# renly/Actor-Critic-Algs-on-Tensorflow

Hardware: AMD Instinct MI355X
Metric: env-steps/sec (whole node) A2C Atari-CNN 32 vec-envs/GPU at 1/2/4/8 MI355X (higher is better)
Workload: dtype bf16; 1 GPU; model=Nature-CNN actor-critic (3 conv + fc512, 1.69M params), global_batch=160, seq_len=5, envs_per_gpu=32, algo=A2C (RMSprop 7e-4, n-step returns, grad-norm 0.5), parallelism=dp1, engine=native, hipgraph=True, dp_schedule=single, grad_bucket_dtype=fp32, dp_world1=False

## Files before the change

### csrc/kernels/cnn_fused.hip

```cpp
#include <cstdlib>

#include "common.h"
#include "cnn_head.h"
#include "launch_api.h"
#include "pong_env.h"

namespace aca {

constexpr int T_THREADS = 256;
constexpr int OBS_BYTES = 4 * 84 * 84;
constexpr int W1_LD = 256 + 8;
constexpr int Y1_ROWS = 400, Y1_C = 32;
constexpr int Y2_ROWS = 81, Y2_C = 64;
constexpr int Y1_LD = 40, Y2_LD = 80;
constexpr int Y3_ROWS = 49, Y3_C = 64;

typedef short short8v __attribute__((ext_vector_type(8)));

__device__ __forceinline__ uint2 u8x4_to_bf16(uint32_t w) {
  uint2 r;
  r.x = (__float_as_uint((float)(w & 0xFF)) >> 16) | (__float_as_uint((float)((w >> 8) & 0xFF)) & 0xFFFF0000u);
  r.y = (__float_as_uint((float)((w >> 16) & 0xFF)) >> 16) | (__float_as_uint((float)(w >> 24)) & 0xFFFF0000u);
  return r;
}
// ... 99 lines not shown
  static constexpr int oia = PART == 1 ? 40 : 0, oib = PART == 0 ? 40 : 84;
  static constexpr int P1 = (c1b - c1a) * 20, T1 = (P1 + 15) / 16;
  static constexpr int P2 = (c2b - c2a) * 9, T2 = (P2 + 15) / 16;
  static constexpr int P3 = (c3b - c3a) * 7, T3 = (P3 + 15) / 16;
  static_assert(c1b <= 20 && ib <= 84 && oia * 84 % 16 == 0, "row ranges");
};
static_assert(EnvRows<-1>::P1 == 400 && EnvRows<-1>::P2 == 81 && EnvRows<-1>::P3 == 49, "whole env");
static_assert(EnvRows<0>::T1 == 15 && EnvRows<1>::T1 == 18 && EnvRows<0>::ib == 52 && EnvRows<1>::ia == 24 &&
              EnvRows<0>::c1b >= EnvRows<0>::o1b && EnvRows<1>::c1a <= EnvRows<1>::o1a &&
              EnvRows<0>::c2b >= EnvRows<0>::o2b && EnvRows<1>::c2a <= EnvRows<1>::o2a &&
              EnvRows<0>::ib >= EnvRows<0>::oib && EnvRows<1>::ia <= EnvRows<1>::oia, "halves own what they compute");
constexpr int E1P_ELEMS = 14 * E1_W * Y1_LD;

template <int PART, bool FRAG = false>
__device__ __forceinline__ void trunk_env_convs(const uint8_t* __restrict__ s_obs8, u16* __restrict__ s_y1,
                                                u16* __restrict__ s_y2, int e, const bf16x8 (&bw)[2][8],
                                                const bf16x8 (&bw2)[16], const u16* __restrict__ W3, float bias0,
                                                float bias1, float bias2, float bias3, u16* __restrict__ y1g,
                                                u16* __restrict__ y2g, u16* __restrict__ y3g, float scale,
                                                uint64_t* __restrict__ stamps = nullptr) {
  using R = EnvRows<PART>;
  constexpr int NW = 4;
  const int tid = threadIdx.x, lane = tid & 63, wid = tid >> 6;
  const int l16 = lane & 15, lg = lane >> 4;
  const int n2 = wid * 16 + l16;
  for (int mt = wid; mt < R::T1; mt += NW) {
    floatx4 acc0 = {0.f, 0.f, 0.f, 0.f}, acc1 = {0.f, 0.f, 0.f, 0.f};
    const int m = min(mt * 16 + l16, R::P1 - 1);
    const int oh = R::c1a + m / 20, ow = m % 20;
#pragma unroll
    for (int ks = 0; ks < 8; ++ks) {
      const int k = ks * 32 + lg * 8;
      const int c = k >> 6, i = (k >> 3) & 7;
      const uint8_t* p = s_obs8 + (c * 84 + oh * 4 + i) * 84 + ow * 4;
      const uint2 lo = u8x4_to_bf16(*reinterpret_cast<const uint32_t*>(p));
      const uint2 hi = u8x4_to_bf16(*reinterpret_cast<const uint32_t*>(p + 4));
      const bf16x8 a = __builtin_bit_cast(bf16x8, make_uint4(lo.x, lo.y, hi.x, hi.y));
      acc0 = __builtin_amdgcn_mfma_f32_16x16x32_bf16(a, bw[0][ks], acc0, 0, 0, 0);
      acc1 = __builtin_amdgcn_mfma_f32_16x16x32_bf16(a, bw[1][ks], acc1, 0, 0, 0);
    }
#pragma unroll
    for (int r = 0; r < 4; ++r) {
      const int row = mt * 16 + lg * 4 + r;
      if (R::P1 % 16 == 0 || row < R::P1) {
        const u16 v0 = f2bf(fmaxf(acc0[r] * scale + bias0, 0.f));
        const u16 v1 = f2bf(fmaxf(acc1[r] * scale + bias1, 0.f));
        const int lr = row / 20, col = row % 20;
        const int px1 = lr * E1_W + col;
        s_y1[px1 * Y1_LD + l16] = v0;
        s_y1[px1 * Y1_LD + 16 + l16] = v1;
        if (PART < 0 || (R::c1a + lr >= R::o1a && R::c1a + lr < R::o1b)) {
          const size_t g = (size_t)e * Y1_ROWS + R::c1a * 20 + row;
          y1g[g * Y1_C + l16] = v0;
          y1g[g * Y1_C + 16 + l16] = v1;
        }
      }
    }
  }
  bf16x8 bw3[18];
  load_w3<FRAG>(W3, bw3);
  __syncthreads();
  stamp(stamps, 5);
  {
    floatx4 acc[R::T2];
#pragma unroll
    for (int mt = 0; mt < R::T2; ++mt) acc[mt] = floatx4{0.f, 0.f, 0.f, 0.f};
#pragma unroll
    for (int ks = 0; ks < 16; ++ks) {
      const int k = ks * 32 + lg * 8;
      const int i = k >> 7, j = (k >> 5) & 3, c0 = k & 31;
#pragma unroll
      for (int mt = 0; mt < R::T2; ++mt) {
        const int m = min(mt * 16 + l16, R::P2 - 1);
        const int oh = m / 9, ow = m - oh * 9;
        const bf16x8 a = *reinterpret_cast<const bf16x8*>(s_y1 + ((oh * 2 + i) * E1_W + ow * 2 + j) * Y1_LD + c0);
        acc[mt] = __builtin_amdgcn_mfma_f32_16x16x32_bf16(a, bw2[ks], acc[mt], 0, 0, 0);
      }
    }
#pragma unroll
    for (int mt = 0; mt < R::T2; ++mt) {
#pragma unroll
      for (int r = 0; r < 4; ++r) {
        const int row = mt * 16 + lg * 4 + r;
        if (row < R::P2) {
          const u16 v = f2bf(fmaxf(acc[mt][r] + bias2, 0.f));
          const int lr = row / 9;
          s_y2[(lr * E2_W + row % 9) * Y2_LD + n2] = v;
          if (PART < 0 || (R::c2a + lr >= R::o2a && R::c2a + lr < R::o2b))
            y2g[((size_t)e * Y2_ROWS + R::c2a * 9 + row) * Y2_C + n2] = v;
        }
      }
    }
  }
  __syncthreads();
  stamp(stamps, 6);
  {
    floatx4 acc[R::T3];
#pragma unroll
    for (int mt = 0; mt < R::T3; ++mt) acc[mt] = floatx4{0.f, 0.f, 0.f, 0.f};
#pragma unroll
    for (int ks = 0; ks < 18; ++ks) {
      const int k = ks * 32 + lg * 8;
      const int i = k / 192, j = (k >> 6) % 3, c0 = k & 63;
#pragma unroll
      for (int mt = 0; mt < R::T3; ++mt) {
        const int m = min(mt * 16 + l16, R::P3 - 1);
        const int oh = m / 7, ow = m - oh * 7;
        const bf16x8 a = *reinterpret_cast<const bf16x8*>(s_y2 + ((oh + i) * E2_W + ow + j) * Y2_LD + c0);
        acc[mt] = __builtin_amdgcn_mfma_f32_16x16x32_bf16(a, bw3[ks], acc[mt], 0, 0, 0);
      }
    }
#pragma unroll
    for (int mt = 0; mt < R::T3; ++mt) {
#pragma unroll
      for (int r = 0; r < 4; ++r) {
        const int row = mt * 16 + lg * 4 + r;
        if (row < R::P3)
          y3g[((size_t)e * Y3_ROWS + R::c3a * 7 + row) * Y3_C + n2] = f2bf(fmaxf(acc[mt][r] + bias3, 0.f));
      }
    }
  }
  stamp(stamps, 7);
}

__device__ __forceinline__ void w1_lds_dma(const u16* __restrict__ W1, u16* dst_lds) {
  const int lane = threadIdx.x & 63, wid = threadIdx.x >> 6, nw = blockDim.x >> 6;
  for (int blk = wid; blk < 16; blk += nw) {
    const int q = blk * 64 + lane, row = q >> 5, lc = (q & 31) ^ (row & 15);
    __builtin_amdgcn_global_load_lds(reinterpret_cast<const uint4*>(W1) + row * 32 + lc,
                                     (__attribute__((address_space(3))) void*)(dst_lds + blk * 512), 16, 0, 0);
  }
}
__device__ __forceinline__ void w1_frags_from_lds(const u16* __restrict__ s_w, bf16x8 (&bw)[2][8]) {
  const int lane = threadIdx.x & 63, l16 = lane & 15, lg = lane >> 4;
#pragma unroll
  for (int nt = 0; nt < 2; ++nt)
#pragma unroll
    for (int ks = 0; ks < 8; ++ks) {
      const int row = nt * 16 + l16, pc = (ks * 4 + lg) ^ (row & 15);
      bw[nt][ks] = *reinterpret_cast<const bf16x8*>(s_w + row * 256 + pc * 8);
    }
}

constexpr int E1T_ELEMS = 20 * 20 * Y1_C;
__device__ __forceinline__ int e1t_addr(int h, int w, int ch) {
  return (h * 20 + (w & 1) * 10 + (w >> 1)) * Y1_C + (((ch >> 3) ^ (((h >> 1) & 1) << 1)) << 3) + (ch & 7);
}
constexpr int OB16_ELEMS = 4 * 84 * 84;
static_assert(E1T_ELEMS + E2_ELEMS <= OB16_ELEMS && Y3_ROWS * Y3_C <= E1T_ELEMS, "y1 + y2 (+ y3) reuse the image");

template <bool FRAG>
__global__ void __launch_bounds__(256) cnn_trunk_fwd_s16_kernel(
    const uint8_t* __restrict__ obs, const u16* __restrict__ W1, const float* __restrict__ b1,
    const u16* __restrict__ W2, const float* __restrict__ b2, const u16* __restrict__ W3,
    const float* __restrict__ b3, u16* __restrict__ y1g, u16* __restrict__ y2g, u16* __restrict__ y3g,
    float scale, uint8_t* __restrict__ shift_out, const int64_t* __restrict__ obs_idx) {
  __shared__ __attribute__((aligned(16))) u16 s_img[OB16_ELEMS];
  u16* const s_y1 = s_img;
  u16* const s_y2 = s_img + E1T_ELEMS;
  u16* const s_y3 = s_img;
  const int e = blockIdx.x;
  const int tid = threadIdx.x, lane = tid & 63, wid = tid >> 6;
  const int l16 = lane & 15, lg = lane >> 4;
  const int n2 = wid * 16 + l16;
  constexpr int NCH = OBS_BYTES / 16, PER = (NCH + 255) / 256;
  const uint4* src = reinterpret_cast<const uint4*>(obs + (size_t)(obs_idx ? obs_idx[e] : e) * OBS_BYTES);
  uint4 v[PER];
#pragma unroll
  for (int u = 0; u < PER; ++u) v[u] = src[min(tid + u * 256, NCH - 1)];
  bf16x8 bw[2][8];
  if constexpr (FRAG) frag_w1(W1, bw);
  else trunk_env_w1(W1, bw);
  const float bias0 = b1[l16], bias1 = b1[16 + l16], bias2 = b2[n2], bias3 = b3[n2];
#pragma unroll
  for (int u = 0; u < PER; ++u) {
    const int i = tid + u * 256;
    if (i < NCH) {
      const uint2 a = u8x4_to_bf16(v[u].x), b = u8x4_to_bf16(v[u].y);
      const uint2 c = u8x4_to_bf16(v[u].z), d = u8x4_to_bf16(v[u].w);
      uint4* dst = reinterpret_cast<uint4*>(s_img) + 2 * i;
      dst[0] = make_uint4(a.x, a.y, b.x, b.y);
      dst[1] = make_uint4(c.x, c.y, d.x, d.y);
      if (shift_out && i >= NCH / 4)
        reinterpret_cast<uint4*>(shift_out + (size_t)e * OBS_BYTES)[i - NCH / 4] = v[u];
    }
  }
  __syncthreads();
  constexpr int MT1 = 7;
  uint32_t yr[MT1][4];
#pragma unroll
  for (int q = 0; q < MT1; ++q) {
    const int mt = wid + 4 * q;
    if (mt < 25) {
      floatx4 acc0 = {0.f, 0.f, 0.f, 0.f}, acc1 = {0.f, 0.f, 0.f, 0.f};
      const int m = mt * 16 + l16;
      const int oh = m / 20, ow = m - oh * 20;
#pragma unroll
      for (int ks = 0; ks < 8; ++ks) {
        const int k = ks * 32 + lg * 8;
        const int c = k >> 6, i = (k >> 3) & 7;
        const u16* p = s_img + (c * 84 + oh * 4 + i) * 84 + ow * 4;
        const uint2 lo = *reinterpret_cast<const uint2*>(p), hi = *reinterpret_cast<const uint2*>(p + 4);
        const bf16x8 a = __builtin_bit_cast(bf16x8, make_uint4(lo.x, lo.y, hi.x, hi.y));
        acc0 = __builtin_amdgcn_mfma_f32_16x16x32_bf16(a, bw[0][ks], acc0, 0, 0, 0);
        acc1 = __builtin_amdgcn_mfma_f32_16x16x32_bf16(a, bw[1][ks], acc1, 0, 0, 0);
      }
#pragma unroll
      for (int r = 0; r < 4; ++r)
        yr[q][r] = (uint32_t)f2bf(fmaxf(acc0[r] * scale + bias0, 0.f)) |
                   ((uint32_t)f2bf(fmaxf(acc1[r] * scale + bias1, 0.f)) << 16);
    }
  }
  bf16x8 bw2[16];
  load_w2<FRAG>(W2, bw2);
  __syncthreads();
#pragma unroll
  for (int q = 0; q < MT1; ++q) {
    const int mt = wid + 4 * q;
    if (mt < 25)
#pragma unroll
      for (int r = 0; r < 4; ++r) {
        const int row = mt * 16 + lg * 4 + r, h = row / 20, w = row - h * 20;
        s_y1[e1t_addr(h, w, l16)] = (u16)(yr[q][r] & 0xFFFFu);
        s_y1[e1t_addr(h, w, 16 + l16)] = (u16)(yr[q][r] >> 16);
      }
  }
  __syncthreads();
  for (int i = tid; i < Y1_ROWS * 4; i += 256) {
    const int p = i >> 2, cq = i & 3, h = p / 20, w = p - h * 20;
    *reinterpret_cast<uint4*>(y1g + ((size_t)e * Y1_ROWS + p) * Y1_C + cq * 8) =
        *reinterpret_cast<const uint4*>(s_y1 + e1t_addr(h, w, cq * 8));
  }
  {
    floatx4 acc[6];
#pragma unroll
    for (int mt = 0; mt < 6; ++mt) acc[mt] = floatx4{0.f, 0.f, 0.f, 0.f};
#pragma unroll
    for (int ks = 0; ks < 16; ++ks) {
      const int k = ks * 32 + lg * 8;
      const int i = k >> 7, j = (k >> 5) & 3, c0 = k & 31;
#pragma unroll
      for (int mt = 0; mt < 6; ++mt) {
        const int m = min(mt * 16 + l16, Y2_ROWS - 1);
        const int oh = m / 9, ow = m - oh * 9;
        const bf16x8 a = *reinterpret_cast<const bf16x8*>(s_y1 + e1t_addr(oh * 2 + i, ow * 2 + j, c0));
        acc[mt] = __builtin_amdgcn_mfma_f32_16x16x32_bf16(a, bw2[ks], acc[mt], 0, 0, 0);
      }
    }
#pragma unroll
    for (int mt = 0; mt < 6; ++mt)
#pragma unroll
      for (int r = 0; r < 4; ++r) {
        const int row = mt * 16 + lg * 4 + r;
        if (row < Y2_ROWS)
          s_y2[((row / 9) * E2_W + row % 9) * Y2_LD + n2] = f2bf(fmaxf(acc[mt][r] + bias2, 0.f));
      }
  }
  bf16x8 bw3[18];
  load_w3<FRAG>(W3, bw3);
  __syncthreads();
  for (int i = tid; i < Y2_ROWS * 8; i += 256) {
    const int p = i >> 3, cq = i & 7;
    *reinterpret_cast<uint4*>(y2g + ((size_t)e * Y2_ROWS + p) * Y2_C + cq * 8) =
        *reinterpret_cast<const uint4*>(s_y2 + ((p / 9) * E2_W + p % 9) * Y2_LD + cq * 8);
  }
  {
    floatx4 acc[4];
#pragma unroll
    for (int mt = 0; mt < 4; ++mt) acc[mt] = floatx4{0.f, 0.f, 0.f, 0.f};
#pragma unroll
    for (int ks = 0; ks < 18; ++ks) {
      const int k = ks * 32 + lg * 8;
      const int i = k / 192, j = (k >> 6) % 3, c0 = k & 63;
#pragma unroll
      for (int mt = 0; mt < 4; ++mt) {
        const int m = min(mt * 16 + l16, Y3_ROWS - 1);
        const int oh = m / 7, ow = m - oh * 7;
        const bf16x8 a = *reinterpret_cast<const bf16x8*>(s_y2 + ((oh + i) * E2_W + ow + j) * Y2_LD + c0);
        acc[mt] = __builtin_amdgcn_mfma_f32_16x16x32_bf16(a, bw3[ks], acc[mt], 0, 0, 0);
      }
    }
#pragma unroll
    for (int mt = 0; mt < 4; ++mt)
#pragma unroll
      for (int r = 0; r < 4; ++r) {
        const int row = mt * 16 + lg * 4 + r;
        if (row < Y3_ROWS) s_y3[row * Y3_C + n2] = f2bf(fmaxf(acc[mt][r] + bias3, 0.f));
      }
  }
  __syncthreads();
  for (int i = tid; i < Y3_ROWS * 8; i += 256)
    reinterpret_cast<uint4*>(y3g + (size_t)e * Y3_ROWS * Y3_C)[i] = reinterpret_cast<const uint4*>(s_y3)[i];
}

constexpr int TR_ROWS = 7;
constexpr int TR_IN_ROWS = 36;
constexpr int TR_C1_ROWS = 8;
constexpr int TR_C1_POS = TR_C1_ROWS * 20;
constexpr int TR_C2_POS = 27;
constexpr int TR_IN_ELEMS = 768 * 16;

__device__ __forceinline__ int tr_y1_own_begin(int r) { return (20 * r + 6) / 7; }

template <int WMODE, bool FRAG = false>
__device__ __forceinline__ void trunk_rows_compute(const u16* __restrict__ s_in, const u16* __restrict__ s_w1,
                                                   u16* __restrict__ s_y1, u16* __restrict__ s_y2, int e, int r,
                                                   const float bias1a, const float bias1b, const float bias2,
                                                   const float bias3, const u16* __restrict__ W2,
                                                   const u16* __restrict__ W3, u16* __restrict__ y1g,
                                                   u16* __restrict__ y2g, u16* __restrict__ y3g, float scale,
                                                   uint64_t* __restrict__ stamps, bf16x8 (&bw2)[16],
                                                   bf16x8 (&bw3)[18]) {
  const int tid = threadIdx.x, lane = tid & 63, wid = tid >> 6;
  const int l16 = lane & 15, lg = lane >> 4;
  const int n2 = wid * 16 + l16;
  if constexpr (WMODE == 0 || WMODE == 2) {
    load_w2<FRAG>(W2, bw2);
  }
  if constexpr (WMODE == 0) {
    load_w3<FRAG>(W3, bw3);
  }

  {
    bf16x8 bw1[2][8];
#pragma unroll
    for (int nt = 0; nt < 2; ++nt)
#pragma unroll
      for (int ks = 0; ks < 8; ++ks)
        bw1[nt][ks] = *reinterpret_cast<const bf16x8*>(s_w1 + (nt * 16 + l16) * W1_LD + ks * 32 + lg * 8);
    const float bias0 = bias1a, bias1 = bias1b;
    auto c1_load = [&](int mt, bf16x8 (&a)[8]) {
      const int m = mt * 16 + l16;
      const int oh = m / 20, ow = m - oh * 20;
#pragma unroll
      for (int ks = 0; ks < 8; ++ks) {
        const int k = ks * 32 + lg * 8;
        const int c = k >> 6, i = (k >> 3) & 7;
        const u16* p = s_in + (c * TR_IN_ROWS + oh * 4 + i) * 84 + ow * 4;
        const uint2 lo = *reinterpret_cast<const uint2*>(p), hi = *reinterpret_cast<const uint2*>(p + 4);
        a[ks] = __builtin_bit_cast(bf16x8, make_uint4(lo.x, lo.y, hi.x, hi.y));
      }
    };
    bf16x8 abuf[2][8];
    c1_load(wid, abuf[0]);
#pragma unroll
    for (int it = 0; it < 3; ++it) {
      const int mt = wid + 4 * it;
      if (mt >= TR_C1_POS / 16) break;
      if (it < 2 && mt + 4 < TR_C1_POS / 16) c1_load(mt + 4, abuf[(it + 1) & 1]);
      const bf16x8 (&a)[8] = abuf[it & 1];
      floatx4 acc0 = {0.f, 0.f, 0.f, 0.f}, acc1 = {0.f, 0.f, 0.f, 0.f};
#pragma unroll
      for (int ks = 0; ks < 8; ++ks) {
        acc0 = __builtin_amdgcn_mfma_f32_16x16x32_bf16(a[ks], bw1[0][ks], acc0, 0, 0, 0);
        acc1 = __builtin_amdgcn_mfma_f32_16x16x32_bf16(a[ks], bw1[1][ks], acc1, 0, 0, 0);
      }
#pragma unroll
      for (int q = 0; q < 4; ++q) {
        const int row = mt * 16 + lg * 4 + q;
        const u16 v0 = f2bf(fmaxf(acc0[q] * scale + bias0, 0.f));
        const u16 v1 = f2bf(fmaxf(acc1[q] * scale + bias1, 0.f));
        s_y1[row * Y1_LD + l16] = v0;
        s_y1[row * Y1_LD + 16 + l16] = v1;
      }
    }
  }
  stamp(stamps, 10);
  if constexpr (WMODE == 1) {
    load_w2<FRAG>(W2, bw2);
  }
  if constexpr (WMODE >= 1) {
    load_w3<FRAG>(W3, bw3);
  }
  __syncthreads();
  stamp(stamps, 2);
  {
    const int n = n2;
    const float bias = bias2;
    floatx4 acc[2];
    acc[0] = floatx4{0.f, 0.f, 0.f, 0.f};
    acc[1] = floatx4{0.f, 0.f, 0.f, 0.f};
    auto c2_load = [&](int ks0, bf16x8 (&a)[4][2]) {
#pragma unroll
      for (int u = 0; u < 4; ++u) {
        const int k = (ks0 + u) * 32 + lg * 8;
        const int i = k >> 7, j = (k >> 5) & 3, c0 = k & 31;
#pragma unroll
        for (int mt = 0; mt < 2; ++mt) {
          const int m = min(mt * 16 + l16, TR_C2_POS - 1);
          const int oh = m / 9, ow = m - oh * 9;
          a[u][mt] = *reinterpret_cast<const bf16x8*>(s_y1 + ((oh * 2 + i) * 20 + ow * 2 + j) * Y1_LD + c0);
        }
      }
    };
    bf16x8 a2[2][4][2];
    c2_load(0, a2[0]);
#pragma unroll
    for (int ch = 0; ch < 4; ++ch) {
      if (ch < 3) c2_load(4 * (ch + 1), a2[(ch + 1) & 1]);
#pragma unroll
      for (int u = 0; u < 4; ++u)
#pragma unroll
        for (int mt = 0; mt < 2; ++mt)
          acc[mt] = __builtin_amdgcn_mfma_f32_16x16x32_bf16(a2[ch & 1][u][mt], bw2[4 * ch + u], acc[mt], 0, 0, 0);
    }
#pragma unroll
    for (int mt = 0; mt < 2; ++mt) {
#pragma unroll
      for (int q = 0; q < 4; ++q) {
        const int row = mt * 16 + lg * 4 + q;
        if (row < TR_C2_POS) s_y2[row * Y2_LD + n] = f2bf(fmaxf(acc[mt][q] + bias, 0.f));
      }
    }
  }
  __syncthreads();
  stamp(stamps, 3);
  {
    const int n = n2;
    const float bias = bias3;
    floatx4 acc = {0.f, 0.f, 0.f, 0.f};
    const int m = min(l16, 6);
    bf16x8 a3[18];
#pragma unroll
    for (int ks = 0; ks < 18; ++ks) {
      const int k = ks * 32 + lg * 8;
      const int i = k / 192, j = (k >> 6) % 3, c0 = k & 63;
      a3[ks] = *reinterpret_cast<const bf16x8*>(s_y2 + (i * 9 + m + j) * Y2_LD + c0);
    }
#pragma unroll
    for (int ks = 0; ks < 18; ++ks) acc = __builtin_amdgcn_mfma_f32_16x16x32_bf16(a3[ks], bw3[ks], acc, 0, 0, 0);
#pragma unroll
    for (int q = 0; q < 4; ++q) {
      const int row = lg * 4 + q;
      const u16 v = f2bf(fmaxf(acc[q] + bias, 0.f));
      if (row < 7) y3g[((size_t)e * Y3_ROWS + r * 7 + row) * Y3_C + n] = v;
    }
  }
  {
    const int p1 = tr_y1_own_begin(r) * 20, p1e = tr_y1_own_begin(r + 1) * 20;
    const int n1 = (p1e - p1) * 4;
    for (int c = tid; c < n1; c += T_THREADS) {
      const int px = p1 + (c >> 2), lp = px - 2 * r * 20, q = (c & 3) * 8;
      *reinterpret_cast<uint4*>(y1g + ((size_t)e * Y1_ROWS + px) * Y1_C + q) =
          *reinterpret_cast<const uint4*>(s_y1 + lp * Y1_LD + q);
    }
    const int n2c = ((r == TR_ROWS - 1) ? 27 : 9) * 8;
    if (tid < n2c) {
      const int lp = tid >> 3, q = (tid & 7) * 8;
      *reinterpret_cast<uint4*>(y2g + ((size_t)e * Y2_ROWS + r * 9 + lp) * Y2_C + q) =
          *reinterpret_cast<const uint4*>(s_y2 + lp * Y2_LD + q);
    }
  }
  if (stamps) {
    stamp(stamps, 4);
    asm volatile("s_waitcnt vmcnt(0)" ::: "memory");
    stamp(stamps, 5);
  }
}


template <bool LATE_W, bool FRAG>
__global__ void __launch_bounds__(T_THREADS) cnn_trunk_rows_kernel(
    const uint8_t* __restrict__ obs, const u16* __restrict__ W1, const float* __restrict__ b1,
    const u16* __restrict__ W2, const float* __restrict__ b2, const u16* __restrict__ W3,
    const float* __restrict__ b3, u16* __restrict__ y1g, u16* __restrict__ y2g, u16* __restrict__ y3g,
    float scale, uint8_t* __restrict__ shift_out, uint8_t* __restrict__ copy_out, uint64_t* __restrict__ stamps) {
  __shared__ __attribute__((aligned(16))) u16 s_in[TR_IN_ELEMS];
  __shared__ __attribute__((aligned(16))) u16 s_w1[32 * W1_LD];
  __shared__ __attribute__((aligned(16))) u16 s_y1[TR_C1_POS * Y1_LD];
  __shared__ __attribute__((aligned(16))) u16 s_y2[TR_C2_POS * Y2_LD];

  const int r = blockIdx.x % TR_ROWS, e = blockIdx.x / TR_ROWS;
  const int tid = threadIdx.x, lane = tid & 63, wid = tid >> 6;
  const int l16 = lane & 15, lg = lane >> 4;
  const int in0 = 8 * r;
  stamp(stamps, 0);

  const int n2 = wid * 16 + l16;
  const float bias1a = b1[l16], bias1b = b1[16 + l16], bias2 = b2[n2], bias3 = b3[n2];
  constexpr int FR_CH = TR_IN_ROWS * 84 / 16;
  constexpr int IN_CH = 4 * FR_CH;
  constexpr int IN_PER = (IN_CH + T_THREADS - 1) / T_THREADS;
  uint4 vo[IN_PER];
  {
    const uint8_t* src = obs + (size_t)e * OBS_BYTES + (size_t)in0 * 84;
#pragma unroll
    for (int u = 0; u < IN_PER; ++u) {
      const int i = min(tid + u * T_THREADS, IN_CH - 1);
      const int f = i / FR_CH, c = i - f * FR_CH;
      vo[u] = *reinterpret_cast<const uint4*>(src + (size_t)f * 84 * 84 + c * 16);
    }
  }
  constexpr int W1_PER = 32 * 256 / 8 / T_THREADS;
  uint4 vw[W1_PER];
#pragma unroll
  for (int u = 0; u < W1_PER; ++u) vw[u] = reinterpret_cast<const uint4*>(W1)[tid + u * T_THREADS];
  {
    uint4* dst = reinterpret_cast<uint4*>(s_in);
#pragma unroll
    for (int u = 0; u < IN_PER; ++u) {
      const int i = tid + u * T_THREADS;
      const uint2 a = u8x4_to_bf16(vo[u].x), b = u8x4_to_bf16(vo[u].y);
      const uint2 c = u8x4_to_bf16(vo[u].z), d = u8x4_to_bf16(vo[u].w);
      dst[2 * i] = make_uint4(a.x, a.y, b.x, b.y);
      dst[2 * i + 1] = make_uint4(c.x, c.y, d.x, d.y);
    }
#pragma unroll
    for (int u = 0; u < W1_PER; ++u) {
      const int i = tid + u * T_THREADS, rr = i / 32, c8 = (i % 32) * 8;
      *reinterpret_cast<uint4*>(s_w1 + rr * W1_LD + c8) = vw[u];
    }
    if (shift_out || copy_out) {
#pragma unroll
      for (int u = 0; u < IN_PER; ++u) {
        const int i = tid + u * T_THREADS;
        const int f = i / FR_CH, c = i - f * FR_CH;
        const bool own = i < IN_CH && c >= 21 * r && c < 21 * r + 63;
        const size_t goff = (size_t)e * OBS_BYTES + (size_t)in0 * 84 + c * 16;
        if (own && copy_out) *reinterpret_cast<uint4*>(copy_out + (size_t)f * 84 * 84 + goff) = vo[u];
        if (own && shift_out && f >= 1)
          *reinterpret_cast<uint4*>(shift_out + (size_t)(f - 1) * 84 * 84 + goff) = vo[u];
      }
    }
    __syncthreads();
  }
  stamp(stamps, 1);
  bf16x8 bw2[16], bw3[18];
  trunk_rows_compute<LATE_W ? 1 : 0, FRAG>(s_in, s_w1, s_y1, s_y2, e, r, bias1a, bias1b, bias2, bias3, W2, W3, y1g,
                                           y2g, y3g, scale, stamps, bw2, bw3);
}

__device__ __forceinline__ void pong_commit_next(const PongIO& io, const PongNext& nx, int e, const PongOut& r,
                                                 int64_t tg_old) {
  nx.tglob[e] = tg_old + 1;
  io.reward[e] = r.rew;
  io.done_out[e] = r.done;
  io.trunc_out[e] = r.trunc;
  if (r.done) {
    atomicAdd(&io.ep_stats[0], r.er);
    atomicAdd(&io.ep_stats[1], 1.0f);
    atomicAdd(&io.ep_stats[2], (float)r.t);
  }
  nx.tsteps[e] = r.done ? 0 : r.t;
  nx.ep_ret[e] = r.done ? 0.0f : r.er;
  float* sp = nx.state + (size_t)e * 8;
  const PongState& q = r.s;
  sp[0] = q.bx; sp[1] = q.by; sp[2] = q.vx; sp[3] = q.vy; sp[4] = q.pa; sp[5] = q.po; sp[6] = q.sa; sp[7] = q.so;
}

template <int A1, bool FRAG>
__global__ void __launch_bounds__(T_THREADS) pong_fused_step_kernel(
    PongIO io, PongNext nx, FcParts fc, u16* __restrict__ h, const u16* __restrict__ Wh,
    const float* __restrict__ bh, float* __restrict__ z_out, int32_t* __restrict__ act, float* __restrict__ logp,
    float* __restrict__ ent, float* __restrict__ vout, int key_shift, uint32_t pseed, const u16* __restrict__ W1,
    const float* __restrict__ b1, const u16* __restrict__ W2, const float* __restrict__ b2,
    const u16* __restrict__ W3, const float* __restrict__ b3, u16* __restrict__ y1g, u16* __restrict__ y2g,
    u16* __restrict__ y3g, float scale, uint8_t* __restrict__ shift_out, uint64_t* __restrict__ stamps) {
  constexpr int A = A1 - 1;
  __shared__ __attribute__((aligned(16))) u16 s_in[TR_IN_ELEMS];
  __shared__ __attribute__((aligned(16))) u16 s_w1[32 * W1_LD];
  __shared__ __attribute__((aligned(16))) u16 s_y1[TR_C1_POS * Y1_LD];
  __shared__ __attribute__((aligned(16))) u16 s_y2[TR_C2_POS * Y2_LD];
  __shared__ float s_acc[4][A1];
  __shared__ PongOut cand[3];
  __shared__ int sh_act;
  const int r = blockIdx.x % TR_ROWS, e = blockIdx.x / TR_ROWS;
  const bool lead = r == 0;
  const int tid = threadIdx.x, lane = tid & 63, wid = tid >> 6, l16 = lane & 15;
  const int in0 = 8 * r;
  stamp(stamps, 0);
  const bool phys = tid >= 64 && tid < 67;
  PongIn pin;
  if (phys) pin = pong_load(io, e);
  const int64_t tg0 = io.tglob[e], id0 = io.env_ids[e];
  const float bhj = bh[lane < A1 ? lane : 0];
  uint32_t wv[A1];
#pragma unroll
  for (int u = 0; u < A1; ++u) wv[u] = reinterpret_cast<const uint32_t*>(Wh)[A1 * tid + u];
  FcH2<16> fch;
  fch.issue(fc.hpart, fc.S, fc.plane_stride, fc.bfc, e, tid);
  const int n2 = wid * 16 + l16;
  const float bias1a = b1[l16], bias1b = b1[16 + l16], bias2 = b2[n2], bias3 = b3[n2];
  constexpr int FR_CH = TR_IN_ROWS * 84 / 16;
  constexpr int IN3_CH = 3 * FR_CH;
  constexpr int IN3_PER = (IN3_CH + T_THREADS - 1) / T_THREADS;
  uint4 vo[IN3_PER];
  {
    const uint8_t* src = io.out + (size_t)e * OBS_BYTES + (size_t)in0 * 84;
#pragma unroll
    for (int u = 0; u < IN3_PER; ++u) {
      const int i = min(tid + u * T_THREADS, IN3_CH - 1);
      const int f = i / FR_CH, c = i - f * FR_CH;
      vo[u] = *reinterpret_cast<const uint4*>(src + (size_t)f * FRAME + c * 16);
    }
  }
  constexpr int W1_PER = 32 * 256 / 8 / T_THREADS;
  uint4 vw[W1_PER];
#pragma unroll
  for (int u = 0; u < W1_PER; ++u) vw[u] = reinterpret_cast<const uint4*>(W1)[tid + u * T_THREADS];
  bf16x8 bw2[16], bw3[18];
  float hf[2];
  if (phys) cand[tid - 64] = pong_advance_in(io, pin, (float)(tid - 65));
  fch.finish(fc.hpart, fc.S, fc.plane_stride, e, tid, lead ? h : nullptr, hf);
  float acc[A1];
#pragma unroll
  for (int j = 0; j < A1; ++j) {
    const uint32_t w0 = wv[j >> 1], w1 = wv[(A1 + j) >> 1];
    const float a0 = __uint_as_float((j & 1) ? (w0 & 0xFFFF0000u) : (w0 << 16));
    const float a1 = __uint_as_float(((A1 + j) & 1) ? (w1 & 0xFFFF0000u) : (w1 << 16));
    acc[j] = wave_sum(hf[0] * a0 + hf[1] * a1);
  }
  if (lane == 0)
#pragma unroll
    for (int j = 0; j < A1; ++j) s_acc[wid][j] = acc[j];
  {
    uint4* dst = reinterpret_cast<uint4*>(s_in);
#pragma unroll
    for (int u = 0; u < IN3_PER; ++u) {
      const int i = tid + u * T_THREADS;
      const uint2 a = u8x4_to_bf16(vo[u].x), b = u8x4_to_bf16(vo[u].y);
      const uint2 c = u8x4_to_bf16(vo[u].z), d = u8x4_to_bf16(vo[u].w);
      dst[2 * i] = make_uint4(a.x, a.y, b.x, b.y);
      dst[2 * i + 1] = make_uint4(c.x, c.y, d.x, d.y);
    }
#pragma unroll
    for (int u = 0; u < W1_PER; ++u) {
      const int i = tid + u * T_THREADS, rr = i / 32, c8 = (i % 32) * 8;
      *reinterpret_cast<uint4*>(s_w1 + rr * W1_LD + c8) = vw[u];
    }
  }
  __syncthreads();
  stamp(stamps, 8);
  if (wid == 0) {
    const int64_t key = tg0 * ((int64_t)1 << key_shift) + id0;
    const int jj = lane < A1 ? lane : 0;
    const float zj = ((s_acc[0][jj] + s_acc[1][jj]) + (s_acc[2][jj] + s_acc[3][jj])) + bhj;
    if (lead && lane < A1) z_out[(size_t)e * A1 + lane] = zj;
    const float value = __int_as_float(__builtin_amdgcn_readlane(__float_as_int(zj), A));
    const CatSample cs = cat_sample<8>(zj, A, lane, pseed, key);
    const int bi = cs.act;
    const float lpa = cs.lpa, H = cs.H;
    if (lane == 0) {
      if (lead) {
        act[e] = bi;
        logp[e] = lpa;
        ent[e] = H;
        vout[e] = value;
      }
      sh_act = bi;
    }
  }
  __syncthreads();
  stamp(stamps, 9);
  load_w2<FRAG>(W2, bw2);
  const PongOut& res = cand[pong_dir_index(sh_act)];
  const bool done = res.done != 0;
  if (lead && tid == 0) pong_commit_next(io, nx, e, res, tg0);
  {
    constexpr int WPR = PW / 4;
    const PongGeom gm = pong_geom(res.s);
    uint32_t* ob = reinterpret_cast<uint32_t*>(io.out + (size_t)e * OBS_BYTES);
    uint32_t* sb = shift_out ? reinterpret_cast<uint32_t*>(shift_out + (size_t)e * OBS_BYTES) : nullptr;
    for (int w = tid; w < TR_IN_ROWS * WPR; w += T_THREADS) {
      const int row = w / WPR, x0 = (w - row * WPR) * 4, y = in0 + row;
      const uint32_t word = pong_word(gm, y, x0);
      const uint2 bw = u8x4_to_bf16(word);
      *reinterpret_cast<uint2*>(s_in + (3 * TR_IN_ROWS + row) * 84 + x0) = bw;
      if (done)
#pragma unroll
        for (int f = 0; f < 3; ++f) *reinterpret_cast<uint2*>(s_in + (f * TR_IN_ROWS + row) * 84 + x0) = bw;
      if (y >= 12 * r && y < 12 * r + 12) {
        const int px = (y * 84 + x0) >> 2;
        ob[(3 * FRAME >> 2) + px] = word;
        if (done)
#pragma unroll
          for (int f = 0; f < 3; ++f) ob[(f * FRAME >> 2) + px] = word;
        if (sb) {
          sb[(2 * FRAME >> 2) + px] = word;
          if (done) {
            sb[px] = word;
            sb[(FRAME >> 2) + px] = word;
          }
        }
      }
    }
    if (sb && !done) {
#pragma unroll
      for (int u = 0; u < IN3_PER; ++u) {
        const int i = tid + u * T_THREADS;
        const int f = i / FR_CH, c = i - f * FR_CH;
        if (i < IN3_CH && f >= 1 && c >= 21 * r && c < 21 * r + 63)
          *reinterpret_cast<uint4*>(shift_out + (size_t)e * OBS_BYTES + (size_t)(f - 1) * FRAME +
                                    (size_t)in0 * 84 + c * 16) = vo[u];
      }
    }
  }
  __syncthreads();
  stamp(stamps, 1);
  trunk_rows_compute<3, FRAG>(s_in, s_w1, s_y1, s_y2, e, r, bias1a, bias1b, bias2, bias3, W2, W3, y1g, y2g, y3g,
                              scale, stamps, bw2, bw3);
}

template <int A1, int PART, bool FRAG>
__device__ __forceinline__ void env_step_body(
    uint8_t* __restrict__ s_obs8, u16* __restrict__ s_y1, float (*s_acc)[A1], PongOut* cand, int* sh_act,
    const PongIO& io, const PongNext& nx, const FcParts& fc, int e, u16* __restrict__ h,
    const u16* __restrict__ Wh, const float* __restrict__ bh, float* __restrict__ z_out, int32_t* __restrict__ act,
    float* __restrict__ logp, float* __restrict__ ent, float* __restrict__ vout, int key_shift, uint32_t pseed,
    const u16* __restrict__ W1, const float* __restrict__ b1, const u16* __restrict__ W2,
    const float* __restrict__ b2, const u16* __restrict__ W3, const float* __restrict__ b3, u16* __restrict__ y1g,
    u16* __restrict__ y2g, u16* __restrict__ y3g, float scale, uint8_t* __restrict__ shift_out,
    uint64_t* __restrict__ stamps) {
  using R = EnvRows<PART>;
  constexpr int A = A1 - 1;
  constexpr bool lead = PART <= 0;
  u16* const s_y2 = reinterpret_cast<u16*>(s_obs8);
  const int tid = threadIdx.x, lane = tid & 63, wid = tid >> 6, l16 = lane & 15;
  const int n2 = wid * 16 + l16;
  stamp(stamps, 0);
  const bool phys = tid >= 64 && tid < 67;
  PongIn pin;
  if (phys) pin = pong_load(io, e);
  const int64_t tg0 = io.tglob[e], id0 = io.env_ids[e];
  const float bhj = bh[lane < A1 ? lane : 0];
  uint32_t wv[A1];
#pragma unroll
  for (int u = 0; u < A1; ++u) wv[u] = reinterpret_cast<const uint32_t*>(Wh)[A1 * tid + u];
  FcH2<16> fch;
  fch.issue(fc.hpart, fc.S, fc.plane_stride, fc.bfc, e, tid);
  obs_rows_dma<R::ia, R::ib>(io.out + (size_t)e * OBS_BYTES, s_obs8);
  w1_lds_dma(W1, s_y1);
  bf16x8 bw[2][8], bw2[16];
  const float bias0 = b1[l16], bias1 = b1[16 + l16], bias2 = b2[n2], bias3 = b3[n2];
  if (phys) cand[tid - 64] = pong_advance_in(io, pin, (float)(tid - 65));
  if (stamps && tid == 64) stamps[(size_t)blockIdx.x * 16 + 10] = __builtin_amdgcn_s_memrealtime();
  float hf[2];
  fch.finish(fc.hpart, fc.S, fc.plane_stride, e, tid, lead ? h : nullptr, hf);
  stamp(stamps, 8);
  float accj[A1];
#pragma unroll
  for (int j = 0; j < A1; ++j) {
    const uint32_t w0 = wv[j >> 1], w1 = wv[(A1 + j) >> 1];
    const float a0 = __uint_as_float((j & 1) ? (w0 & 0xFFFF0000u) : (w0 << 16));
    const float a1 = __uint_as_float(((A1 + j) & 1) ? (w1 & 0xFFFF0000u) : (w1 << 16));
    accj[j] = wave_sum(hf[0] * a0 + hf[1] * a1);
  }
  if (lane == 0)
#pragma unroll
    for (int j = 0; j < A1; ++j) s_acc[wid][j] = accj[j];
  stamp(stamps, 9);
  __syncthreads();
  stamp(stamps, 1);
  asm volatile("s_waitcnt vmcnt(0)" ::: "memory");
  if (wid == 0) {
    const int64_t key = tg0 * ((int64_t)1 << key_shift) + id0;
    const int jj = lane < A1 ? lane : 0;
    const float zj = ((s_acc[0][jj] + s_acc[1][jj]) + (s_acc[2][jj] + s_acc[3][jj])) + bhj;
    if (lead && lane < A1) z_out[(size_t)e * A1 + lane] = zj;
    const float value = __int_as_float(__builtin_amdgcn_readlane(__float_as_int(zj), A));
    const CatSample cs = cat_sample<8>(zj, A, lane, pseed, key);
    const int bi = cs.act;
    const float lpa = cs.lpa, H = cs.H;
    if (lane == 0) {
      if (lead) {
        act[e] = bi;
        logp[e] = lpa;
        ent[e] = H;
        vout[e] = value;
      }
      *sh_act = bi;
    }
  }
  __syncthreads();
  stamp(stamps, 2);
  w1_frags_from_lds(s_y1, bw);
  load_w2<FRAG>(W2, bw2);
  const PongOut& res = cand[pong_dir_index(*sh_act)];
  const bool done = res.done != 0;
  if (tid == 0) {
    if constexpr (PART < 0) pong_commit(io, e, res, tg0);
    else if constexpr (PART == 0) pong_commit_next(io, nx, e, res, tg0);
  }
  {
    constexpr int WPR = PW / 4, NWORDS = PH * WPR;
    const PongGeom gm = pong_geom(res.s);
    uint32_t* ob = reinterpret_cast<uint32_t*>(io.out + (size_t)e * OBS_BYTES);
    uint32_t* sw = reinterpret_cast<uint32_t*>(s_obs8);
    for (int w = R::ia * WPR + tid; w < R::ib * WPR; w += 256) {
      const int y = w / WPR, x0 = (w - y * WPR) * 4;
      const uint32_t word = pong_word(gm, y, x0);
      const bool own = PART < 0 || (y >= R::oia && y < R::oib);
      sw[3 * NWORDS + w] = word;
      if (own) ob[3 * NWORDS + w] = word;
      if (done)
#pragma unroll
        for (int f = 0; f < 3; ++f) {
          sw[f * NWORDS + w] = word;
          if (own) ob[f * NWORDS + w] = word;
        }
    }
  }
  __syncthreads();
  stamp(stamps, 3);
  if (shift_out) {
    uint4* so = reinterpret_cast<uint4*>(shift_out + (size_t)e * OBS_BYTES);
    const uint4* si = reinterpret_cast<const uint4*>(s_obs8);
    constexpr int FC = FRAME / 16, C0 = R::oia * 84 / 16, NC = (R::oib - R::oia) * 84 / 16;
    for (int i = tid; i < 3 * NC; i += 256) {
      const int f = i / NC, c = C0 + i - f * NC;
      so[f * FC + c] = si[(f + 1) * FC + c];
    }
  }
  stamp(stamps, 4);
  trunk_env_convs<PART, FRAG>(s_obs8, s_y1, s_y2, e, bw, bw2, W3, bias0, bias1, bias2, bias3, y1g, y2g, y3g, scale,
                              stamps);
}

template <int A1, int SPLIT, bool FRAG>
__global__ void __launch_bounds__(256) pong_fused_env_step_kernel(
    PongIO io, PongNext nx, FcParts fc, u16* __restrict__ h, const u16* __restrict__ Wh, const float* __restrict__ bh,
    float* __restrict__ z_out, int32_t* __restrict__ act, float* __restrict__ logp, float* __restrict__ ent,
    float* __restrict__ vout, int key_shift, uint32_t pseed, const u16* __restrict__ W1,
    const float* __restrict__ b1, const u16* __restrict__ W2, const float* __restrict__ b2,
    const u16* __restrict__ W3, const float* __restrict__ b3, u16* __restrict__ y1g, u16* __restrict__ y2g,
    u16* __restrict__ y3g, float scale, uint8_t* __restrict__ shift_out, uint64_t* __restrict__ stamps) {
  __shared__ __attribute__((aligned(16))) uint8_t s_obs8[TP_OBS_PAD];
  __shared__ __attribute__((aligned(16))) u16 s_y1[SPLIT == 1 ? E1_ELEMS : E1P_ELEMS];
  __shared__ float s_acc[4][A1];
  __shared__ PongOut cand[3];
  __shared__ int sh_act;
#define ACA_ENV_BODY(PART, E)                                                                                    \
  env_step_body<A1, PART, FRAG>(s_obs8, s_y1, s_acc, cand, &sh_act, io, nx, fc, E, h, Wh, bh, z_out, act, logp,     \
                                ent, vout, key_shift, pseed, W1, b1, W2, b2, W3, b3, y1g, y2g, y3g, scale, shift_out, stamps)
  if constexpr (SPLIT == 1) {
    ACA_ENV_BODY(-1, blockIdx.x);
  } else {
    if (blockIdx.x & 1) ACA_ENV_BODY(1, blockIdx.x >> 1);
    else ACA_ENV_BODY(0, blockIdx.x >> 1);
  }
#undef ACA_ENV_BODY
}

__device__ __forceinline__ int div9(int n) { return (int)(((unsigned)n * 57u) >> 9); }
__device__ __forceinline__ int div10(int n) { return (int)(((unsigned)n * 205u) >> 11); }
__device__ __forceinline__ int div7(int n) { return (int)(((unsigned)n * 37u) >> 8); }
constexpr int BW_LDW3 = 64;
constexpr int BW_LDW2 = 32;
constexpr int BW_PS = 80;
constexpr int BW_P3H = 11, BW_P3W = 17;
constexpr int BW_P2H = 11, BW_P2W = 18;
constexpr int BW_RW = 576 * BW_LDW3;
constexpr int BW_P3E = BW_P3H * BW_P3W * BW_PS;
constexpr int BW_M2E = 81 * 64;
constexpr int BW_P2E = BW_P2H * BW_P2W * BW_PS;
static_assert(400 * 32 + 32 <= BW_P3E + BW_M2E, "dy1 staging (+ its discard slots) aliases the dy3 image + y2 mask");
static_assert(1024 * BW_LDW2 <= BW_RW, "W2 rows fit the W3 region");
static_assert(BW_P3W % 8 == 9 % 8 && BW_P2W % 8 == 10 % 8 && BW_PS == 80, "conflict-free image geometry");
__device__ __forceinline__ int bw_sw3(int r) { return (((r >> 1) & 1) << 1) | (((r >> 3) & 1) << 2); }
__device__ __forceinline__ int bw_sw2(int r) { return ((r >> 3) & 1) << 1; }
template <int H, int W, int LO, int N, int NT>
__device__ __forceinline__ void bw_zero_border(u16* img) {
  const uint4 z4 = make_uint4(0u, 0u, 0u, 0u);
  for (int c = threadIdx.x; c < H * W * 8; c += NT) {
    const int px = c >> 3, part = c & 7, pa = px / W, pb = px - pa * W;
    if (pa < LO || pa >= LO + N || pb < LO || pb >= LO + N)
      *reinterpret_cast<uint4*>(img + px * BW_PS + part * 8) = z4;
  }
}

__device__ __forceinline__ float bf_lane(const uint4& v, int e) {
  const uint32_t w = e < 2 ? v.x : (e < 4 ? v.y : (e < 6 ? v.z : v.w));
  return __uint_as_float((e & 1) ? (w & 0xFFFF0000u) : (w << 16));
}
__device__ __forceinline__ uint32_t mask_pair(uint32_t w, uint32_t m) {
  const uint32_t lo = (__uint_as_float(m << 16) > 0.f) ? 0x0000FFFFu : 0u;
  const uint32_t hi = (__uint_as_float(m & 0xFFFF0000u) > 0.f) ? 0xFFFF0000u : 0u;
  return w & (lo | hi);
}

template <int SW>
__device__ __forceinline__ bf16x8 tr_frag_sw(const u16* rows, int ld, int col0, int lane) {
  const int lr16 = lane & 15, lg = lane >> 4, q = lr16 >> 2, p = lr16 & 3;
  const int r0 = lg * 8 + q, r1 = r0 + 4, col = col0 + 4 * p;
  const int s0 = SW == 3 ? bw_sw3(r0) : bw_sw2(r0), s1 = SW == 3 ? bw_sw3(r1) : bw_sw2(r1);
  const u16* p0 = rows + r0 * ld + ((((col >> 3) ^ s0) << 3) | (col & 7));
  const u16* p1 = rows + r1 * ld + ((((col >> 3) ^ s1) << 3) | (col & 7));
  typedef short short4x __attribute__((ext_vector_type(4)));
  typedef __attribute__((address_space(3))) short4x lds4;
  const short4x lo = __builtin_amdgcn_ds_read_tr16_b64_v4i16((lds4*)(p0));
  const short4x hi = __builtin_amdgcn_ds_read_tr16_b64_v4i16((lds4*)(p1));
  const short8v v = {lo[0], lo[1], lo[2], lo[3], hi[0], hi[1], hi[2], hi[3]};
  return __builtin_bit_cast(bf16x8, v);
}

__device__ __forceinline__ bf16x8 tr_frag(const u16* rows, int ld, int col0, int lane) {
  const int lr16 = lane & 15, lg = lane >> 4, q = lr16 >> 2, p = lr16 & 3;
  const u16* p0 = rows + (lg * 8 + q) * ld + col0 + 4 * p;
  const u16* p1 = rows + (lg * 8 + 4 + q) * ld + col0 + 4 * p;
  typedef short short4x __attribute__((ext_vector_type(4)));
  typedef __attribute__((address_space(3))) short4x lds4;
  const short4x lo = __builtin_amdgcn_ds_read_tr16_b64_v4i16((lds4*)(p0));
  const short4x hi = __builtin_amdgcn_ds_read_tr16_b64_v4i16((lds4*)(p1));
  const short8v v = {lo[0], lo[1], lo[2], lo[3], hi[0], hi[1], hi[2], hi[3]};
  return __builtin_bit_cast(bf16x8, v);
}

constexpr int BW_T = 512;
constexpr int BW_FR = 4 * 84 * 84;
static_assert(BW_FR + 8 <= BW_RW, "the bf16 frames + a zero chunk fit the weight region");
static_assert(416 * 32 <= BW_P3E + BW_M2E, "dy1 rows + 16 zero padding rows (13 k-steps of 32) fit the staging");

__global__ void __launch_bounds__(BW_T) cnn_trunk_bwd_kernel(
    const u16* __restrict__ dy3g, const u16* __restrict__ W3, const u16* __restrict__ y2g,
    const u16* __restrict__ W2, const u16* __restrict__ y1g, u16* __restrict__ dy2g, u16* __restrict__ dy1g,
    float* __restrict__ biasp, uint64_t* __restrict__ stamps) {
  __shared__ __attribute__((aligned(16))) u16 s_w[BW_RW];
  __shared__ __attribute__((aligned(16))) u16 s_p3m2[BW_P3E + BW_M2E];
  __shared__ __attribute__((aligned(16))) u16 s_p2[BW_P2E];
  __shared__ float s_red[8 * 128 + 8 * 32];
  u16* const s_p3 = s_p3m2;
  u16* const s_m2 = s_p3m2 + BW_P3E;
  u16* const s_d1 = s_p3m2;
  const int b = blockIdx.x;
  const int tid = threadIdx.x, lane = tid & 63, wid = tid >> 6;
  const int l16 = lane & 15, lg = lane >> 4;
  stamp(stamps, 0);

  {
    constexpr int W3_CH = 576 * 8, W3_PER = W3_CH / BW_T;
    constexpr int M2_CH = 81 * 8;
    constexpr int M2_PER = (M2_CH + BW_T - 1) / BW_T;
    uint4 vw[W3_PER], vm[M2_PER];
    const uint4 vp = *reinterpret_cast<const uint4*>(dy3g + (size_t)b * 49 * 64 + min(tid, 391) * 8);
#pragma unroll
    for (int u = 0; u < W3_PER; ++u) {
      const int c = tid + u * BW_T, k = c >> 3, part = c & 7;
      const int t = k >> 6, o = k & 63;
      vw[u] = *reinterpret_cast<const uint4*>(W3 + o * 576 + t * 64 + part * 8);
    }
#pragma unroll
    for (int u = 0; u < M2_PER; ++u) {
      const int c = min(tid + u * BW_T, M2_CH - 1);
      vm[u] = *reinterpret_cast<const uint4*>(y2g + (size_t)b * 81 * 64 + c * 8);
    }
    if (tid < 392) {
      const int px = tid >> 3, pa = px / 7, pb = px - pa * 7;
      *reinterpret_cast<uint4*>(s_p3 + ((pa + 2) * BW_P3W + pb + 2) * BW_PS + (tid & 7) * 8) = vp;
    }
    bw_zero_border<BW_P3H, BW_P3W, 2, 7, BW_T>(s_p3);
#pragma unroll
    for (int u = 0; u < W3_PER; ++u) {
      const int c = tid + u * BW_T, k = c >> 3;
      *reinterpret_cast<uint4*>(s_w + k * BW_LDW3 + (((c & 7) ^ bw_sw3(k)) << 3)) = vw[u];
    }
#pragma unroll
    for (int u = 0; u < M2_PER; ++u) {
      const int c = tid + u * BW_T;
      if (c < M2_CH) *reinterpret_cast<uint4*>(s_m2 + c * 8) = vm[u];
    }
    bw_zero_border<BW_P2H, BW_P2W, 1, 9, BW_T>(s_p2);
  }
  static_assert(64 * 512 / 8 / BW_T == 8, "W2 prefetch is written out for 8 chunks per thread");
#define ACA_W2_LD(u) const uint4 vw2_##u = *reinterpret_cast<const uint4*>(W2 + (tid + (u) * BW_T) * 8);
  ACA_W2_LD(0) ACA_W2_LD(1) ACA_W2_LD(2) ACA_W2_LD(3) ACA_W2_LD(4) ACA_W2_LD(5) ACA_W2_LD(6) ACA_W2_LD(7)
#undef ACA_W2_LD
  constexpr int M1_CH = 400 * 4, M1_PER = (M1_CH + BW_T - 1) / BW_T;
  uint4 vm1[M1_PER];
#pragma unroll
  for (int u = 0; u < M1_PER; ++u) {
    const int c = min(tid + u * BW_T, M1_CH - 1);
    vm1[u] = *reinterpret_cast<const uint4*>(y1g + (size_t)b * 400 * 32 + c * 8);
  }
  __syncthreads();
  stamp(stamps, 1);

  {
    const int n0 = (wid & 3) * 16, mh = (wid >> 2) * 3;
    floatx4 acc[3];
#pragma unroll
    for (int mt = 0; mt < 3; ++mt) acc[mt] = floatx4{0.f, 0.f, 0.f, 0.f};
    constexpr int P3_LO = 2 * BW_P3W + 2;
    int pb[3];
#pragma unroll
    for (int mt = 0; mt < 3; ++mt) {
      const int m = min((mh + mt) * 16 + l16, 80);
      const int a = div9(m), c = m - a * 9;
      pb[mt] = ((a + 2) * BW_P3W + (c + 2) - P3_LO) * BW_PS + lg * 8;
    }
#pragma unroll
    for (int ks = 0; ks < 18; ++ks) {
      const int t = ks >> 1, ti = t / 3, tj = t - ti * 3;
      const int off = (P3_LO - ti * BW_P3W - tj) * BW_PS + (ks & 1) * 32;
      const bf16x8 bf = tr_frag_sw<3>(s_w + ks * 32 * BW_LDW3, BW_LDW3, n0, lane);
#pragma unroll
      for (int mt = 0; mt < 3; ++mt) {
        const bf16x8 af = *reinterpret_cast<const bf16x8*>(s_p3 + pb[mt] + off);
        acc[mt] = __builtin_amdgcn_mfma_f32_16x16x32_bf16(af, bf, acc[mt], 0, 0, 0);
      }
    }
    const int n = n0 + l16;
#pragma unroll
    for (int mt = 0; mt < 3; ++mt)
#pragma unroll
// ... 594 lines not shown
```

Baseline: 1.082 million env-steps/s.

## Split conv1 into pre/post phases to overlap with action sampling

```diff
diff --git a/csrc/kernels/cnn_fused.hip b/csrc/kernels/cnn_fused.hip
--- a/csrc/kernels/cnn_fused.hip
+++ b/csrc/kernels/cnn_fused.hip
@@ -425,6 +425,96 @@
 
 __device__ __forceinline__ int tr_y1_own_begin(int r) { return (20 * r + 6) / 7; }
 
+constexpr int C1_KS_PRE = 6;
+template <bool LIGHT0>
+__device__ __forceinline__ int c1_tiles(int wid) {
+  return LIGHT0 ? (wid == 0 ? 1 : 3) : (wid < 2 ? 3 : 2);
+}
+template <bool LIGHT0>
+__device__ __forceinline__ int c1_tile(int wid, int it) {
+  return LIGHT0 ? (wid == 0 ? TR_C1_POS / 16 - 1 : wid - 1 + 3 * it) : wid + 4 * it;
+}
+__device__ __forceinline__ bf16x8 c1_afrag(const u16* __restrict__ s_in, int mt, int ks, int l16, int lg) {
+  const int m = mt * 16 + l16;
+  const int oh = m / 20, ow = m - oh * 20;
+  const int k = ks * 32 + lg * 8;
+  const int c = k >> 6, i = (k >> 3) & 7;
+  const u16* p = s_in + (c * TR_IN_ROWS + oh * 4 + i) * 84 + ow * 4;
+  const uint2 lo = *reinterpret_cast<const uint2*>(p), hi = *reinterpret_cast<const uint2*>(p + 4);
+  return __builtin_bit_cast(bf16x8, make_uint4(lo.x, lo.y, hi.x, hi.y));
+}
+__device__ __forceinline__ bf16x8 c1_bfrag(const u16* __restrict__ s_w1, int nt, int ks, int l16, int lg) {
+  return *reinterpret_cast<const bf16x8*>(s_w1 + (nt * 16 + l16) * W1_LD + ks * 32 + lg * 8);
+}
+
+template <bool LIGHT0>
+__device__ __forceinline__ void conv1_pre(const u16* __restrict__ s_in, const u16* __restrict__ s_w1,
+                                          floatx4 (&acc)[3][2]) {
+  const int lane = threadIdx.x & 63, l16 = lane & 15, lg = lane >> 4;
+  const int wid = __builtin_amdgcn_readfirstlane(threadIdx.x >> 6), nt = c1_tiles<LIGHT0>(wid);
+  bf16x8 bw1[2][C1_KS_PRE];
+#pragma unroll
+  for (int n = 0; n < 2; ++n)
+#pragma unroll
+    for (int ks = 0; ks < C1_KS_PRE; ++ks) bw1[n][ks] = c1_bfrag(s_w1, n, ks, l16, lg);
+#pragma unroll
+  for (int it = 0; it < 3; ++it) acc[it][0] = acc[it][1] = floatx4{0.f, 0.f, 0.f, 0.f};
+  bf16x8 abuf[2][C1_KS_PRE];
+  auto load = [&](int it, bf16x8 (&a)[C1_KS_PRE]) {
+    const int mt = c1_tile<LIGHT0>(wid, it);
+#pragma unroll
+    for (int ks = 0; ks < C1_KS_PRE; ++ks) a[ks] = c1_afrag(s_in, mt, ks, l16, lg);
+  };
+  load(0, abuf[0]);
+#pragma unroll
+  for (int it = 0; it < 3; ++it) {
+    if (it >= nt) break;
+    if (it < 2 && it + 1 < nt) load(it + 1, abuf[(it + 1) & 1]);
+    const bf16x8 (&a)[C1_KS_PRE] = abuf[it & 1];
+#pragma unroll
+    for (int ks = 0; ks < C1_KS_PRE; ++ks) {
+      acc[it][0] = __builtin_amdgcn_mfma_f32_16x16x32_bf16(a[ks], bw1[0][ks], acc[it][0], 0, 0, 0);
+      acc[it][1] = __builtin_amdgcn_mfma_f32_16x16x32_bf16(a[ks], bw1[1][ks], acc[it][1], 0, 0, 0);
+    }
+  }
+}
+
+template <bool LIGHT0>
+__device__ __forceinline__ void conv1_post(const u16* __restrict__ s_in, const u16* __restrict__ s_w1,
+                                           u16* __restrict__ s_y1, floatx4 (&acc)[3][2], float scale, float bias0,
+                                           float bias1) {
+  const int lane = threadIdx.x & 63, l16 = lane & 15, lg = lane >> 4;
+  const int wid = __builtin_amdgcn_readfirstlane(threadIdx.x >> 6), nt = c1_tiles<LIGHT0>(wid);
+  bf16x8 bw1[2][2], a[3][2];
+#pragma unroll
+  for (int n = 0; n < 2; ++n)
+#pragma unroll
+    for (int u = 0; u < 2; ++u) bw1[n][u] = c1_bfrag(s_w1, n, C1_KS_PRE + u, l16, lg);
+#pragma unroll
+  for (int it = 0; it < 3; ++it)
+    if (it < nt)
+#pragma unroll
+      for (int u = 0; u < 2; ++u) a[it][u] = c1_afrag(s_in, c1_tile<LIGHT0>(wid, it), C1_KS_PRE + u, l16, lg);
+#pragma unroll
+  for (int it = 0; it < 3; ++it) {
+    if (it >= nt) break;
+    const int mt = c1_tile<LIGHT0>(wid, it);
+#pragma unroll
+    for (int u = 0; u < 2; ++u) {
+      acc[it][0] = __builtin_amdgcn_mfma_f32_16x16x32_bf16(a[it][u], bw1[0][u], acc[it][0], 0, 0, 0);
+      acc[it][1] = __builtin_amdgcn_mfma_f32_16x16x32_bf16(a[it][u], bw1[1][u], acc[it][1], 0, 0, 0);
+    }
+#pragma unroll
+    for (int q = 0; q < 4; ++q) {
+      const int row = mt * 16 + lg * 4 + q;
+      const u16 v0 = f2bf(fmaxf(acc[it][0][q] * scale + bias0, 0.f));
+      const u16 v1 = f2bf(fmaxf(acc[it][1][q] * scale + bias1, 0.f));
+      s_y1[row * Y1_LD + l16] = v0;
+      s_y1[row * Y1_LD + 16 + l16] = v1;
+    }
+  }
+}
+
 template <int WMODE, bool FRAG = false>
 __device__ __forceinline__ void trunk_rows_compute(const u16* __restrict__ s_in, const u16* __restrict__ s_w1,
                                                    u16* __restrict__ s_y1, u16* __restrict__ s_y2, int e, int r,
@@ -433,7 +523,7 @@
                                                    const u16* __restrict__ W3, u16* __restrict__ y1g,
                                                    u16* __restrict__ y2g, u16* __restrict__ y3g, float scale,
                                                    uint64_t* __restrict__ stamps, bf16x8 (&bw2)[16],
-                                                   bf16x8 (&bw3)[18]) {
+                                                   bf16x8 (&bw3)[18], floatx4 (&acc1)[3][2]) {
   const int tid = threadIdx.x, lane = tid & 63, wid = tid >> 6;
   const int l16 = lane & 15, lg = lane >> 4;
   const int n2 = wid * 16 + l16;
@@ -444,50 +534,8 @@
     load_w3<FRAG>(W3, bw3);
   }
 
-  {
-    bf16x8 bw1[2][8];
-#pragma unroll
-    for (int nt = 0; nt < 2; ++nt)
-#pragma unroll
-      for (int ks = 0; ks < 8; ++ks)
-        bw1[nt][ks] = *reinterpret_cast<const bf16x8*>(s_w1 + (nt * 16 + l16) * W1_LD + ks * 32 + lg * 8);
-    const float bias0 = bias1a, bias1 = bias1b;
-    auto c1_load = [&](int mt, bf16x8 (&a)[8]) {
-      const int m = mt * 16 + l16;
-      const int oh = m / 20, ow = m - oh * 20;
-#pragma unroll
-      for (int ks = 0; ks < 8; ++ks) {
-        const int k = ks * 32 + lg * 8;
-        const int c = k >> 6, i = (k >> 3) & 7;
-        const u16* p = s_in + (c * TR_IN_ROWS + oh * 4 + i) * 84 + ow * 4;
-        const uint2 lo = *reinterpret_cast<const uint2*>(p), hi = *reinterpret_cast<const uint2*>(p + 4);
-        a[ks] = __builtin_bit_cast(bf16x8, make_uint4(lo.x, lo.y, hi.x, hi.y));
-      }
-    };
-    bf16x8 abuf[2][8];
-    c1_load(wid, abuf[0]);
-#pragma unroll
-    for (int it = 0; it < 3; ++it) {
-      const int mt = wid + 4 * it;
-      if (mt >= TR_C1_POS / 16) break;
-      if (it < 2 && mt + 4 < TR_C1_POS / 16) c1_load(mt + 4, abuf[(it + 1) & 1]);
-      const bf16x8 (&a)[8] = abuf[it & 1];
-      floatx4 acc0 = {0.f, 0.f, 0.f, 0.f}, acc1 = {0.f, 0.f, 0.f, 0.f};
-#pragma unroll
-      for (int ks = 0; ks < 8; ++ks) {
-        acc0 = __builtin_amdgcn_mfma_f32_16x16x32_bf16(a[ks], bw1[0][ks], acc0, 0, 0, 0);
-        acc1 = __builtin_amdgcn_mfma_f32_16x16x32_bf16(a[ks], bw1[1][ks], acc1, 0, 0, 0);
-      }
-#pragma unroll
-      for (int q = 0; q < 4; ++q) {
-        const int row = mt * 16 + lg * 4 + q;
-        const u16 v0 = f2bf(fmaxf(acc0[q] * scale + bias0, 0.f));
-        const u16 v1 = f2bf(fmaxf(acc1[q] * scale + bias1, 0.f));
-        s_y1[row * Y1_LD + l16] = v0;
-        s_y1[row * Y1_LD + 16 + l16] = v1;
-      }
-    }
-  }
+  if constexpr (WMODE != 3) conv1_pre<false>(s_in, s_w1, acc1);
+  conv1_post<WMODE == 3>(s_in, s_w1, s_y1, acc1, scale, bias1a, bias1b);
   stamp(stamps, 10);
   if constexpr (WMODE == 1) {
     load_w2<FRAG>(W2, bw2);
@@ -649,8 +697,9 @@
   }
   stamp(stamps, 1);
   bf16x8 bw2[16], bw3[18];
+  floatx4 acc1[3][2];
   trunk_rows_compute<LATE_W ? 1 : 0, FRAG>(s_in, s_w1, s_y1, s_y2, e, r, bias1a, bias1b, bias2, bias3, W2, W3, y1g,
-                                           y2g, y3g, scale, stamps, bw2, bw3);
+                                           y2g, y3g, scale, stamps, bw2, bw3, acc1);
 }
 
 __device__ __forceinline__ void pong_commit_next(const PongIO& io, const PongNext& nx, int e, const PongOut& r,
@@ -773,11 +822,16 @@
       sh_act = bi;
     }
   }
+  stamp(stamps, 11);
+  const bool wave0 = __builtin_amdgcn_readfirstlane(wid) == 0;
+  floatx4 acc1[3][2];
+  if (!wave0) conv1_pre<true>(s_in, s_w1, acc1);
+  if (stamps && tid == 64) stamps[(size_t)blockIdx.x * 16 + 13] = __builtin_amdgcn_s_memrealtime();
   __syncthreads();
   stamp(stamps, 9);
   load_w2<FRAG>(W2, bw2);
   const PongOut& res = cand[pong_dir_index(sh_act)];
-  const bool done = res.done != 0;
+  const bool done = __builtin_amdgcn_readfirstlane(res.done) != 0;
   if (lead && tid == 0) pong_commit_next(io, nx, e, res, tg0);
   {
     constexpr int WPR = PW / 4;
@@ -820,8 +874,10 @@
   }
   __syncthreads();
   stamp(stamps, 1);
+  if (done || wave0) conv1_pre<true>(s_in, s_w1, acc1);
+  stamp(stamps, 12);
   trunk_rows_compute<3, FRAG>(s_in, s_w1, s_y1, s_y2, e, r, bias1a, bias1b, bias2, bias3, W2, W3, y1g, y2g, y3g,
-                              scale, stamps, bw2, bw3);
+                              scale, stamps, bw2, bw3, acc1);
 }
 
 template <int A1, int PART, bool FRAG>
```

Result: no change. 1.083 million env-steps/s, median of 2 (+0.0%).
